# thobotics/geometry_rl

Measured on AMD Instinct MI355X. Metric: policy-update steps/sec, HEPi 4096 envs x 128 steps, higher is better.
Workload: dtype f32 storage/accumulate, bf16x3 products (three bf16 MFMAs per f32 product)

## Files before the change

### geometry_rl_amd/csrc/edge_conv16.hip

```cpp
#include "grl_tile16.h"
#include "grl_wimg.h"
#include <cstdlib>

namespace {

constexpr int C = 64, O = 16;

constexpr int E16_WAVES = 4, E16_THREADS = 64 * E16_WAVES;
constexpr int E16_WGS = 3;
constexpr int LD1 = WI_LD1, LD2 = WI_LD2;

struct Edge16Params {
  const st_t* x_in;
  const float* pos_src;
  const float* pos_dst;
  const int* rowptr;
  const int* e_src;
  const int* e_dst;
  const int* erow;
  const float* grid, *W1, *b1, *W2, *b2, *Wk;
  int n_anchor, n_edges, dim;
  int anchor_is_dst;
  int per_edge;
  int npw;
  const int* split;
  const void* wimg;
};

GRL_DEVINL void load_w16(ChainW16& s, const Edge16Params& p) {
  if (p.wimg) {
    copy_image<E16_THREADS>(&s, p.wimg, (int)sizeof(ChainW16));
    return;
  }
  stage16<14, 32, E16_THREADS>(s.W1h, s.W1l, p.W1, LD1);
  stage16<64, 64, E16_THREADS>(s.W2h, s.W2l, p.W2, LD2);
  stage16<64, 64, E16_THREADS>(s.Wkh, s.Wkl, p.Wk, LD2);
  stage_chain16_small<E16_THREADS>(s, p.b1, p.b2, p.grid);
}

template <int KS, bool FENCED = true, class Epi>
GRL_DEVINL void group16(const unsigned short* whi, const unsigned short* wlo, const bf16x8 (&xh)[KS], const bf16x8 (&xl)[KS], f32x4v acc,
                        Epi&& epi) {
  bf16x8 wh[KS], wl[KS];
#pragma unroll
  for (int s = 0; s < KS; ++s) {
    wh[s] = *reinterpret_cast<const bf16x8*>(whi + 32 * s);
    GRL_LO(wl[s] = *reinterpret_cast<const bf16x8*>(wlo + 32 * s);)
  }
  if (FENCED) __builtin_amdgcn_sched_barrier(0);
#pragma unroll
  for (int s = 0; s < KS; ++s) {
    acc = mfma16(wh[s], xh[s], acc);
    GRL_LO(acc = mfma16(wl[s], xh[s], acc);)
    GRL_LO(acc = mfma16(wh[s], xl[s], acc);)
  }
  epi(acc);
  if (FENCED) __builtin_amdgcn_sched_barrier(0);
}


template <class KEpi>
GRL_DEVINL void chain16(const ChainW16& w, float a, float b, int r, int g, KEpi&& k_epi) {
  const float aa = a * a, ab = a * b, bb = b * b;
  float4 phi;
  if (g == 0) phi = make_float4(a, b, aa, ab);
  else if (g == 1) phi = make_float4(ab, bb, aa * a, aa * b);
  else if (g == 2) phi = make_float4(ab * a, ab * b, ab * a, ab * b);
  else phi = make_float4(bb * a, bb * b, 0.f, 0.f);
  bf16x8 ph[1], pl[1];
  split_pair(phi, make_float4(0.f, 0.f, 0.f, 0.f), ph[0], pl[0]);
  float4 g1[4], g2[4];
#pragma unroll
  for (int nt = 0; nt < 4; ++nt) {
    const float4 bq = *reinterpret_cast<const float4*>(w.b1s + 16 * nt + 4 * g);
    group16<1>(w.W1h + (16 * nt + r) * LD1 + 8 * g, w.W1l + (16 * nt + r) * LD1 + 8 * g, ph, pl, f32x4v{bq.x, bq.y, bq.z, bq.w},
               [&](const f32x4v& acc) { g1[nt] = gelu4(v4(acc)); });
  }
  bf16x8 xh[2], xl[2];
  split_pair(g1[0], g1[1], xh[0], xl[0]);
  split_pair(g1[2], g1[3], xh[1], xl[1]);
  __builtin_amdgcn_sched_barrier(0);
#pragma unroll
  for (int nt = 0; nt < 4; ++nt) {
    const float4 bq = *reinterpret_cast<const float4*>(w.b2s + 16 * nt + 4 * g);
    group16<2>(w.W2h + (16 * nt + r) * LD2 + 8 * g, w.W2l + (16 * nt + r) * LD2 + 8 * g, xh, xl, f32x4v{bq.x, bq.y, bq.z, bq.w},
               [&](const f32x4v& acc) { g2[nt] = gelu4(v4(acc)); });
  }
  bf16x8 yh[2], yl[2];
  split_pair(g2[0], g2[1], yh[0], yl[0]);
  split_pair(g2[2], g2[3], yh[1], yl[1]);
  __builtin_amdgcn_sched_barrier(0);
#pragma unroll
  for (int nt = 0; nt < 4; ++nt)
    group16<2>(w.Wkh + (16 * nt + r) * LD2 + 8 * g, w.Wkl + (16 * nt + r) * LD2 + 8 * g, yh, yl, f32x4v{0.f, 0.f, 0.f, 0.f},
               [&](const f32x4v& acc) { k_epi(nt, v4(acc)); });
}

#if GRL_PREC
struct ChainRegs {
  bf16x8 w2[4][2], wk[4][2];
  GRL_LO(bf16x8 w2l[4][2]; bf16x8 wkl[4][2];)
};
GRL_DEVINL void chain_regs_load(ChainRegs& cr, const ChainW16& w, int r, int g) {
#pragma unroll
  for (int nt = 0; nt < 4; ++nt) {
#pragma unroll
    for (int s = 0; s < 2; ++s) {
      cr.w2[nt][s] = *reinterpret_cast<const bf16x8*>(w.W2h + (16 * nt + r) * LD2 + 8 * g + 32 * s);
      cr.wk[nt][s] = *reinterpret_cast<const bf16x8*>(w.Wkh + (16 * nt + r) * LD2 + 8 * g + 32 * s);
      GRL_LO(cr.w2l[nt][s] = *reinterpret_cast<const bf16x8*>(w.W2l + (16 * nt + r) * LD2 + 8 * g + 32 * s);)
      GRL_LO(cr.wkl[nt][s] = *reinterpret_cast<const bf16x8*>(w.Wkl + (16 * nt + r) * LD2 + 8 * g + 32 * s);)
    }
  }
}
template <class KEpi>
GRL_DEVINL void chain16_resident(const ChainRegs& cr, const ChainW16& w, float a, float b, int r, int g, KEpi&& k_epi) {
  __builtin_amdgcn_sched_barrier(0);
  float4 b1q[4], b2q[4];
  bf16x8 w1[4];
  GRL_LO(bf16x8 w1l[4];)
#pragma unroll
  for (int nt = 0; nt < 4; ++nt) {
    w1[nt] = *reinterpret_cast<const bf16x8*>(w.W1h + (16 * nt + r) * LD1 + 8 * g);
    GRL_LO(w1l[nt] = *reinterpret_cast<const bf16x8*>(w.W1l + (16 * nt + r) * LD1 + 8 * g);)
    b1q[nt] = *reinterpret_cast<const float4*>(w.b1s + 16 * nt + 4 * g);
    b2q[nt] = *reinterpret_cast<const float4*>(w.b2s + 16 * nt + 4 * g);
  }
  const float aa = a * a, ab = a * b, bb = b * b;
  float4 phi;
  if (g == 0) phi = make_float4(a, b, aa, ab);
  else if (g == 1) phi = make_float4(ab, bb, aa * a, aa * b);
  else if (g == 2) phi = make_float4(ab * a, ab * b, ab * a, ab * b);
  else phi = make_float4(bb * a, bb * b, 0.f, 0.f);
  bf16x8 ph, pl;
  split_pair(phi, make_float4(0.f, 0.f, 0.f, 0.f), ph, pl);
  f32x4v c[4];
  float4 g1[4], g2[4];
#pragma unroll
  for (int nt = 0; nt < 4; ++nt) c[nt] = mfma16(w1[nt], ph, f32x4v{b1q[nt].x, b1q[nt].y, b1q[nt].z, b1q[nt].w});
#if !GRL_PREC
#pragma unroll
  for (int nt = 0; nt < 4; ++nt) c[nt] = mfma16(w1l[nt], ph, c[nt]);
#pragma unroll
  for (int nt = 0; nt < 4; ++nt) c[nt] = mfma16(w1[nt], pl, c[nt]);
#endif
#pragma unroll
  for (int nt = 0; nt < 4; ++nt) g1[nt] = gelu4(v4(c[nt]));
  bf16x8 xh[2], xl[2];
  split_pair(g1[0], g1[1], xh[0], xl[0]);
  split_pair(g1[2], g1[3], xh[1], xl[1]);
#pragma unroll
  for (int nt = 0; nt < 4; ++nt) c[nt] = f32x4v{b2q[nt].x, b2q[nt].y, b2q[nt].z, b2q[nt].w};
#pragma unroll
  for (int s = 0; s < 2; ++s) {
#pragma unroll
    for (int nt = 0; nt < 4; ++nt) c[nt] = mfma16(cr.w2[nt][s], xh[s], c[nt]);
#if !GRL_PREC
#pragma unroll
    for (int nt = 0; nt < 4; ++nt) c[nt] = mfma16(cr.w2l[nt][s], xh[s], c[nt]);
#pragma unroll
    for (int nt = 0; nt < 4; ++nt) c[nt] = mfma16(cr.w2[nt][s], xl[s], c[nt]);
#endif
  }
#pragma unroll
  for (int nt = 0; nt < 4; ++nt) g2[nt] = gelu4(v4(c[nt]));
  bf16x8 yh[2], yl[2];
  split_pair(g2[0], g2[1], yh[0], yl[0]);
  split_pair(g2[2], g2[3], yh[1], yl[1]);
#pragma unroll
  for (int nt = 0; nt < 4; ++nt) c[nt] = f32x4v{0.f, 0.f, 0.f, 0.f};
#pragma unroll
  for (int s = 0; s < 2; ++s) {
#pragma unroll
    for (int nt = 0; nt < 4; ++nt) c[nt] = mfma16(cr.wk[nt][s], yh[s], c[nt]);
#if !GRL_PREC
#pragma unroll
    for (int nt = 0; nt < 4; ++nt) c[nt] = mfma16(cr.wkl[nt][s], yh[s], c[nt]);
#pragma unroll
    for (int nt = 0; nt < 4; ++nt) c[nt] = mfma16(cr.wk[nt][s], yl[s], c[nt]);
#endif
  }
#pragma unroll
  for (int nt = 0; nt < 4; ++nt) k_epi(nt, v4(c[nt]));
  __builtin_amdgcn_sched_barrier(0);
}
#define E16_CHAIN(S, A, B, R, G, EPI) chain16_resident(cregs, S, A, B, R, G, EPI)
#else
#define E16_CHAIN chain16
#endif
constexpr int NPW_MAX = 16;

template <int MODE>
__global__ __launch_bounds__(E16_THREADS, E16_WGS) void edge16_kernel(Edge16Params p, st_t* __restrict__ out, const st_t* __restrict__ dres) {
  extern __shared__ __attribute__((aligned(16))) float smem_raw[];
  ChainW16& s = *reinterpret_cast<ChainW16*>(smem_raw);
  load_w16(s, p);
  __syncthreads();
  const int lane = threadIdx.x & 63, wave = threadIdx.x >> 6, r = lane & 15, g = lane >> 4;
  const float gx = s.grid_s[3 * r], gy = s.grid_s[3 * r + 1], gz = s.grid_s[3 * r + 2];
#if GRL_PREC
  ChainRegs cregs;
  chain_regs_load(cregs, s, r, g);
#endif
  const int* e_other = p.anchor_is_dst ? p.e_src : p.e_dst;
  const float* pos_anchor = p.anchor_is_dst ? p.pos_dst : p.pos_src;
  const float* pos_other = p.anchor_is_dst ? p.pos_src : p.pos_dst;
  const int NPW = p.split ? NPW_MAX : p.npw;
  const int n_chunks = (p.n_anchor + NPW - 1) / NPW;
  const int slot = blockIdx.x * E16_WAVES + wave;
  const int n_lo = p.split ? p.split[slot] : 0, n_hi = p.split ? p.split[slot + 1] : p.n_anchor;
  for (int it = 0;; ++it) {
    int n0, nn;
    if (p.split) {
      n0 = n_lo + it * NPW_MAX;
      if (n0 >= n_hi) break;
      nn = min(NPW_MAX, n_hi - n0);
    } else {
      const int chunk = slot + it * (int)gridDim.x * E16_WAVES;
      if (chunk >= n_chunks) break;
      n0 = chunk * NPW;
      nn = min(NPW, p.n_anchor - n0);
    }
    const int rp = p.rowptr[n0 + min(lane, nn)];
    const int an = n0 + min(lane, nn - 1);
    const float pax = pos_anchor[3 * an], pay = pos_anchor[3 * an + 1], paz = pos_anchor[3 * an + 2];
    const int E0 = __builtin_amdgcn_readlane(rp, 0), E1 = __builtin_amdgcn_readlane(rp, nn);
    int node = 0;
    int node_end = __builtin_amdgcn_readlane(rp, 1);
    float4 acc[4];
#pragma unroll
    for (int t = 0; t < 4; ++t) acc[t] = make_float4(0.f, 0.f, 0.f, 0.f);
    auto flush = [&](int j) {
      if (MODE == 2) return;
      st_t* o = out + ((size_t)(n0 + j) * O + r) * C + 4 * g;
#pragma unroll
      for (int t = 0; t < 4; ++t) {
        float4 v = acc[t];
        if (MODE == 1 && dres) v = f4_add_pk(v, ld4(dres + ((size_t)(n0 + j) * O + r) * C + 4 * g + 16 * t));
        st4(o + 16 * t, v);
        acc[t] = make_float4(0.f, 0.f, 0.f, 0.f);
      }
    };
    for (int eb = E0; eb < E1; eb += 64) {
      const int ee = min(eb + lane, E1 - 1);
      const int oth = e_other[ee];
      const int xrow = p.per_edge ? (p.erow ? p.erow[ee] : ee) : oth;
      const float pox = pos_other[3 * oth], poy = pos_other[3 * oth + 1], poz = pos_other[3 * oth + 2];
      const int nb = min(64, E1 - eb);
#pragma unroll 1
      for (int k = 0; k < nb; ++k) {
        const int e = eb + k;
        while (e >= node_end) {
          flush(node);
          ++node;
          node_end = __builtin_amdgcn_readlane(rp, node + 1);
        }
        const int row_in = __builtin_amdgcn_readlane(xrow, k);
        const st_t* xs = p.x_in + ((size_t)row_in * O + r) * C + 4 * g;
        float4 xv[4];
#pragma unroll
        for (int t = 0; t < 4; ++t)
          xv[t] = ld4(xs + 16 * t);
        float dx = __builtin_bit_cast(float, __builtin_amdgcn_readlane(__builtin_bit_cast(int, pox), k)) -
                   __builtin_bit_cast(float, __builtin_amdgcn_readlane(__builtin_bit_cast(int, pax), node));
        float dy = __builtin_bit_cast(float, __builtin_amdgcn_readlane(__builtin_bit_cast(int, poy), k)) -
                   __builtin_bit_cast(float, __builtin_amdgcn_readlane(__builtin_bit_cast(int, pay), node));
        float dz = __builtin_bit_cast(float, __builtin_amdgcn_readlane(__builtin_bit_cast(int, poz), k)) -
                   __builtin_bit_cast(float, __builtin_amdgcn_readlane(__builtin_bit_cast(int, paz), node));
        if (!p.anchor_is_dst) { dx = -dx; dy = -dy; dz = -dz; }
        if (p.dim == 2) dz = 0.f;
        const float a = dx * gx + dy * gy + dz * gz;
        dx -= a * gx; dy -= a * gy; dz -= a * gz;
        const float b = sqrtf(dx * dx + dy * dy + dz * dz);
        st_t* mrow = MODE == 2 ? out + ((size_t)e * O + r) * C + 4 * g : nullptr;
        E16_CHAIN(s, a, b, r, g, [&](int nt, const float4& kq) {
          const float4 m = f4_mul_pk(kq, xv[nt]);
          if (MODE == 2) st4(mrow + 16 * nt, m);
          else acc[nt] = f4_add_pk(acc[nt], m);
        });
      }
    }
    for (; node < nn; ++node) flush(node);
  }
}

struct Stage16 {
  unsigned short Ah[STG], Al[STG];
  unsigned short Bh[STG], Bl[STG];
};
struct Bwd16Smem {
  Edge16Image img;
  Stage16 st[4];
};
constexpr int BWD16_PARTIAL = 64 * 14 + 64 + 64 * 64 + 64 + 64 * 64;

template <int NTK>
struct RFrags {
  bf16x8 ah[2], al[2], bh[NTK], bl[NTK];
};
template <int NTK>
GRL_DEVINL void rowred_load(const Stage16& st, int lane, RFrags<NTK>& f) {
#pragma unroll
  for (int t = 0; t < 2; ++t) {
    f.ah[t] = tr_frag(st.Ah, t, lane);
    GRL_LO(f.al[t] = tr_frag(st.Al, t, lane);)
  }
#pragma unroll
  for (int t = 0; t < NTK; ++t) {
    f.bh[t] = tr_frag(st.Bh, t, lane);
    GRL_LO(f.bl[t] = tr_frag(st.Bl, t, lane);)
  }
}
template <int NTK>
GRL_DEVINL void rowred_mma(const RFrags<NTK>& f, f32x16 (&acc)[2][NTK]) {
#pragma unroll
  for (int tn = 0; tn < 2; ++tn)
#pragma unroll
    for (int tk = 0; tk < NTK; ++tk) {
      mfma32_acc(f.ah[tn], f.bh[tk], acc[tn][tk]);
      GRL_LO(mfma32_acc(f.al[tn], f.bh[tk], acc[tn][tk]);)
      GRL_LO(mfma32_acc(f.ah[tn], f.bl[tk], acc[tn][tk]);)
    }
}

GRL_DEVINL void gelu_both4_pk(const float4& x, float4& gv, float4& gpv) {
  v2f g0, g1, d0, d1;
  gelu_pair<true>(v2f{x.x, x.y}, g0, d0);
  gelu_pair<true>(v2f{x.z, x.w}, g1, d1);
  gv = make_float4(g0.x, g0.y, g1.x, g1.y);
  gpv = make_float4(d0.x, d0.y, d1.x, d1.y);
}
#ifdef GRL_B16_PHASE
__device__ unsigned long long g_b16phase[16];
#define B16_PH(i) do { const unsigned long long t_ = __builtin_amdgcn_s_memtime(); ph_[i] += t_ - tl_; tl_ = t_; } while (0)
#else
#define B16_PH(i)
#endif
struct Bwd16Params {
  Edge16Params e;
  const st_t* x_src;
  const st_t* dres;
  st_t* dx_src;
  float* partial;
  const int* split;
};

__global__ __launch_bounds__(256, 1) void edge_bwd16_kernel(Bwd16Params bp) {
  extern __shared__ __attribute__((aligned(16))) float smem_raw[];
  Bwd16Smem& sm = *reinterpret_cast<Bwd16Smem*>(smem_raw);
  const Edge16Params& p = bp.e;
  if (p.wimg) {
    copy_image<256>(&sm.img, p.wimg, (int)sizeof(Edge16Image));
  } else {
    stage16<14, 32, 256>(sm.img.w.W1h, sm.img.w.W1l, p.W1, LD1);
    stage16<64, 64, 256>(sm.img.w.W2h, sm.img.w.W2l, p.W2, LD2);
    stage16<64, 64, 256>(sm.img.w.Wkh, sm.img.w.Wkl, p.Wk, LD2);
    stage16<64, 64, 256, true>(sm.img.WkTh, sm.img.WkTl, p.Wk, LD2);
    stage16<64, 64, 256, true>(sm.img.W2Th, sm.img.W2Tl, p.W2, LD2);
    stage_chain16_small<256>(sm.img.w, p.b1, p.b2, p.grid);
  }
  const int lane = threadIdx.x & 63, wave = threadIdx.x >> 6, r = lane & 15, g = lane >> 4;
  Stage16& st = sm.st[wave];
  for (int i = lane; i < STG / 2; i += 64) {
    reinterpret_cast<unsigned*>(st.Ah)[i] = 0u; reinterpret_cast<unsigned*>(st.Al)[i] = 0u;
    reinterpret_cast<unsigned*>(st.Bh)[i] = 0u; reinterpret_cast<unsigned*>(st.Bl)[i] = 0u;
  }
  __syncthreads();
  const ChainW16& w = sm.img.w;
  const float gx = w.grid_s[3 * r], gy = w.grid_s[3 * r + 1], gz = w.grid_s[3 * r + 2];
  const bool g0 = g == 0, g1_ = g == 1, g2_ = g == 2;

#if GRL_PREC
  struct LayerFrags { bf16x8 h[4][2]; };
  auto lf_load = [&](LayerFrags& f, const unsigned short* img) {
#pragma unroll
    for (int nt = 0; nt < 4; ++nt)
#pragma unroll
      for (int s_ = 0; s_ < 2; ++s_) f.h[nt][s_] = *reinterpret_cast<const bf16x8*>(img + (16 * nt + r) * LD2 + 8 * g + 32 * s_);
  };
  LayerFrags bufA, bufB;
  lf_load(bufA, w.W2h);
  lf_load(bufB, w.Wkh);
#else
  struct LayerFrags { bf16x8 h[4][2], l[4][2]; };
  auto lf_load = [&](LayerFrags& f, const unsigned short* imh, const unsigned short* iml) {
#pragma unroll
    for (int nt = 0; nt < 4; ++nt)
#pragma unroll
      for (int s_ = 0; s_ < 2; ++s_) {
        f.h[nt][s_] = *reinterpret_cast<const bf16x8*>(imh + (16 * nt + r) * LD2 + 8 * g + 32 * s_);
        f.l[nt][s_] = *reinterpret_cast<const bf16x8*>(iml + (16 * nt + r) * LD2 + 8 * g + 32 * s_);
      }
  };
  LayerFrags buf;
  lf_load(buf, w.W2h, w.W2l);
#endif
  f32x16 accK[2][2], accA[2][2], accB[2][1];
#pragma unroll
  for (int a_ = 0; a_ < 2; ++a_) {
    accB[a_][0] = zero16();
#pragma unroll
    for (int b_ = 0; b_ < 2; ++b_) { accK[a_][b_] = zero16(); accA[a_][b_] = zero16(); }
  }
  float4 db2[4];
#pragma unroll
  for (int t = 0; t < 4; ++t) db2[t] = make_float4(0.f, 0.f, 0.f, 0.f);

#ifdef GRL_B16_PHASE
  unsigned long long ph_[12] = {0}, tl_ = __builtin_amdgcn_s_memtime();
#endif
  const int NPW = bp.split ? NPW_MAX : p.npw;
  const int slot = blockIdx.x * 4 + wave;
  const int n_lo = bp.split ? bp.split[slot] : 0, n_hi = bp.split ? bp.split[slot + 1] : p.n_anchor;
  const int n_chunks = (p.n_anchor + NPW - 1) / NPW;
#pragma unroll 1
  for (int it = 0;; ++it) {
    int n0, nn;
    if (bp.split) {
      n0 = n_lo + it * NPW_MAX;
      if (n0 >= n_hi) break;
      nn = min(NPW_MAX, n_hi - n0);
    } else {
      const int chunk = slot + it * (int)gridDim.x * 4;
// ... 287 lines not shown
#if GRL_PREC
        materialise();
#endif
        bf16x8 kh[2], kl[2];
        RFrags<2> rf;
        layer64(4, yh, yl, [&](int nt, const f32x4v& c) { acc[nt] = f4_add_pk(acc[nt], f4_mul_pk(v4(c), dv[nt])); },
                [&]() {
                  split_pair(f4_mul_pk(dv[0], xv[0]), f4_mul_pk(dv[1], xv[1]), kh[0], kl[0]);
                  split_pair(f4_mul_pk(dv[2], xv[2]), f4_mul_pk(dv[3], xv[3]), kh[1], kl[1]);
                  stage_put<2>(st.Ah, st.Al, kh, kl, r, g);
                  stage_put<2>(st.Bh, st.Bl, yh, yl, r, g);
                  rowred_load<2>(st, lane, rf);
                });
        B16_PH(3);
        bf16x8 zh[2], zl[2];
        {
          float4 dz2[4];
          layer64(8, kh, kl,
                  [&](int nt, const f32x4v& c) {
                    dz2[nt] = f4_mul_pk(v4(c), gp2[nt]);
                    db2[nt] = f4_add_pk(db2[nt], dz2[nt]);
                  },
                  [&]() {
                    rowred_mma<2>(rf, accK);
                    split_pair(dz2[0], dz2[1], zh[0], zl[0]);
                    split_pair(dz2[2], dz2[3], zh[1], zl[1]);
                  });
        }
        B16_PH(4);
        stage_put<2>(st.Ah, st.Al, zh, zl, r, g);
        stage_put<2>(st.Bh, st.Bl, xh, xl, r, g);
        rowred_load<2>(st, lane, rf);
        bf16x8 uh[2], ul[2];
        {
          float4 dz1[4];
          layer64(12, zh, zl, [&](int nt, const f32x4v& c) { dz1[nt] = f4_mul_pk(v4(c), gp1[nt]); },
                  [&]() {
                    rowred_mma<2>(rf, accA);
                    split_pair(dz1[0], dz1[1], uh[0], ul[0]);
                    split_pair(dz1[2], dz1[3], uh[1], ul[1]);
                  });
        }
        B16_PH(5);
        stage_put<2>(st.Ah, st.Al, uh, ul, r, g);
        {
          const u32x4 h4 = __builtin_bit_cast(u32x4, ph[0]);
          *reinterpret_cast<uint2*>(st.Bh + stg_off(r, g)) = make_uint2(h4[0], h4[1]);
          *reinterpret_cast<uint2*>(st.Bh + stg_off(r, 4 + g)) = make_uint2(0u, 0u);
#if !GRL_PREC
          const u32x4 l4 = __builtin_bit_cast(u32x4, pl[0]);
          *reinterpret_cast<uint2*>(st.Bl + stg_off(r, g)) = make_uint2(l4[0], l4[1]);
          *reinterpret_cast<uint2*>(st.Bl + stg_off(r, 4 + g)) = make_uint2(0u, 0u);
#endif
        }
        B16_PH(6);
#undef BAR
      }
    }
    flush(node);
    skip_empty_run(node + 1, nn);
  }

  {
    RFrags<1> rf1;
    rowred_load<1>(st, lane, rf1);
    rowred_mma<1>(rf1, accB);
  }
#ifdef GRL_B16_PHASE
  if (lane == 0 && wave == 0)
    for (int i = 0; i < 12; ++i) atomicAdd(&g_b16phase[i], ph_[i]);
#endif
  constexpr int NACC = 10 * 16 + 16;
  float* fold = smem_raw;
  acc_drain(accB[0][0], accB[1][0], accA[0][0], accA[0][1], accA[1][0], accA[1][1], accK[0][0], accK[0][1], accK[1][0], accK[1][1]);
  auto visit = [&](auto&& f) {
    int k = 0;
#pragma unroll
    for (int a_ = 0; a_ < 2; ++a_) {
#pragma unroll
      for (int i = 0; i < 16; ++i) accB[a_][0][i] = f(accB[a_][0][i], k++);
#pragma unroll
      for (int b_ = 0; b_ < 2; ++b_)
#pragma unroll
        for (int i = 0; i < 16; ++i) { accA[a_][b_][i] = f(accA[a_][b_][i], k++); accK[a_][b_][i] = f(accK[a_][b_][i], k++); }
    }
#pragma unroll
    for (int t = 0; t < 4; ++t) {
      db2[t].x = f(db2[t].x, k++); db2[t].y = f(db2[t].y, k++); db2[t].z = f(db2[t].z, k++); db2[t].w = f(db2[t].w, k++);
    }
  };
  __syncthreads();
  if (wave & 1) visit([&](float v_, int k) { fold[((wave >> 1) * NACC + k) * 64 + lane] = v_; return v_; });
  __syncthreads();
  if (!(wave & 1)) visit([&](float v_, int k) { return v_ + fold[((wave >> 1) * NACC + k) * 64 + lane]; });
  __syncthreads();
  if (wave == 2) visit([&](float v_, int k) { fold[k * 64 + lane] = v_; return v_; });
  __syncthreads();
  if (wave != 0) return;
  visit([&](float v_, int k) { return v_ + fold[k * 64 + lane]; });
  const int j = lane & 31, hh = lane >> 5;
  float* out = bp.partial + (size_t)blockIdx.x * BWD16_PARTIAL;
  float* oW1 = out, *ob1 = out + 64 * 14, *oW2 = ob1 + 64, *ob2 = oW2 + 64 * 64, *oWk = ob2 + 64;
#pragma unroll
  for (int nt = 0; nt < 2; ++nt)
#pragma unroll
    for (int rho = 0; rho < 16; ++rho) {
      const int n = 32 * nt + (rho & 3) + 8 * (rho >> 2) + 4 * hh;
      if (j < 14) oW1[n * 14 + j] = accB[nt][0][rho];
      if (j == 14) ob1[n] = accB[nt][0][rho];
#pragma unroll
      for (int kt = 0; kt < 2; ++kt) {
        oW2[n * 64 + 32 * kt + j] = accA[nt][kt][rho];
        oWk[n * 64 + 32 * kt + j] = accK[nt][kt][rho];
      }
    }
#pragma unroll
  for (int t = 0; t < 4; ++t) {
    float v[4] = {db2[t].x, db2[t].y, db2[t].z, db2[t].w};
#pragma unroll
    for (int u = 0; u < 4; ++u) {
      float x = v[u];
      x += __shfl_xor(x, 1, 64); x += __shfl_xor(x, 2, 64); x += __shfl_xor(x, 4, 64); x += __shfl_xor(x, 8, 64);
      if (r == 0) ob2[16 * t + 4 * g + u] = x;
    }
  }
}

}

extern "C" {

#if !GRL_PREC
static_assert(E16_WAVES == 4, "grl_edge_fwd_slots (edge_conv.hip) counts four wave slots per workgroup");
int grl_edge_fwd_chunk_nodes(int n_dst) {
  if (n_dst < 0) return 256 * E16_WGS;
  const int npw = n_dst / (4 * 256 * E16_WAVES * E16_WGS);
  return npw < 1 ? 1 : (npw > NPW_MAX ? NPW_MAX : npw);
}
int grl_edge_bwd_chunk_nodes(int n_src) {
  const int npw = n_src / (4 * 1024);
  return npw < 1 ? 1 : (npw > NPW_MAX ? NPW_MAX : npw);
}
#else
int grl_edge_fwd_chunk_nodes(int n_dst);
int grl_edge_bwd_chunk_nodes(int n_src);
#endif

int GRL_ENTRY(grl_edge16_launch)(int mode, const st_t* x_in, const float* pos_src, const float* pos_dst, const int* rowptr, const int* e_src,
                                 const int* e_dst, const int* erow, int per_edge, int n_anchor, int n_edges, int anchor_is_dst,
                                 const float* grid, int dim, const float* W1, const float* b1, const float* W2, const float* b2,
                                 const float* Wk, st_t* out, const st_t* dres, const int* split, int n_slots, const void* wimg,
                                 hipStream_t stream) {
  if (n_anchor <= 0) return 0;
  int npw = grl_edge_fwd_chunk_nodes(n_anchor);
  Edge16Params p{x_in, pos_src, pos_dst, rowptr, e_src, e_dst, erow, grid, W1, b1, W2, b2, Wk, n_anchor, n_edges, dim, anchor_is_dst,
                 per_edge, npw, (mode == 0 && split && n_slots >= E16_WAVES && n_slots % E16_WAVES == 0) ? split : nullptr, wimg};
  const int n_chunks = (n_anchor + npw - 1) / npw;
  int blocks = p.split ? n_slots / E16_WAVES : (n_chunks + E16_WAVES - 1) / E16_WAVES;
  int cap = 256 * E16_WGS;
  if (blocks > cap && !p.split) blocks = cap;
  if (blocks < 1) blocks = 1;
  const size_t smem = sizeof(ChainW16);
  GRL_ONCE(hipFuncSetAttribute((const void*)edge16_kernel<0>, hipFuncAttributeMaxDynamicSharedMemorySize, (int)sizeof(ChainW16));
           hipFuncSetAttribute((const void*)edge16_kernel<2>, hipFuncAttributeMaxDynamicSharedMemorySize, (int)sizeof(ChainW16)));
  if (mode == 0) hipLaunchKernelGGL(edge16_kernel<0>, dim3(blocks), dim3(E16_THREADS), smem, stream, p, out, dres);
  else if (mode == 1) return -4;
  else hipLaunchKernelGGL(edge16_kernel<2>, dim3(blocks), dim3(E16_THREADS), smem, stream, p, out, dres);
  GRL_CHECK_LAUNCH();
  return 0;
}

int GRL_ENTRY(grl_edge_bwd16_launch)(const st_t* x_src, const st_t* dmsg, const float* pos_src, const float* pos_dst, const int* rowptr_s,
                                     const int* src_s, const int* dst_s, const int* erow, int per_edge, int n_src, int n_edges,
                                     const float* grid, int dim, const float* W1, const float* b1, const float* W2, const float* b2,
                                     const float* Wk, const st_t* dres, st_t* dx_src, float* partial, int blocks, const int* split,
                                     const void* wimg, hipStream_t stream) {
  const int npw = grl_edge_bwd_chunk_nodes(n_src);
  Bwd16Params bp{{dmsg, pos_src, pos_dst, rowptr_s, src_s, dst_s, erow, grid, W1, b1, W2, b2, Wk, n_src, n_edges, dim, 0, per_edge, npw,
                  nullptr, wimg},
                 x_src, dres, dx_src, partial, split};
  static_assert(sizeof(Bwd16Smem) > 80 * 1024, "edge_bwd16_kernel must not share a CU with a second workgroup");
  GRL_ONCE(hipFuncSetAttribute((const void*)edge_bwd16_kernel, hipFuncAttributeMaxDynamicSharedMemorySize, (int)sizeof(Bwd16Smem)));
  hipLaunchKernelGGL(edge_bwd16_kernel, dim3(blocks), dim3(256), sizeof(Bwd16Smem), stream, bp);
  GRL_CHECK_LAUNCH();
  return 0;
}

#if defined(GRL_B16_PHASE)
int GRL_ENTRY(grl_edge_bwd16_phase_read)(unsigned long long* out16, int reset) {
  hipMemcpyFromSymbol(out16, HIP_SYMBOL(g_b16phase), sizeof(unsigned long long) * 16);
  if (reset) { unsigned long long z[16] = {0}; hipMemcpyToSymbol(HIP_SYMBOL(g_b16phase), z, sizeof(z)); }
  return 0;
}
#endif

}
```

### geometry_rl_amd/csrc/grl_common.h

```cpp
#pragma once
#include <hip/hip_runtime.h>
#include <stdint.h>

typedef float f32x16 __attribute__((ext_vector_type(16)));

#define GRL_DEVINL __device__ __forceinline__

#define GRL_LD(K) ((K) + 4)

GRL_DEVINL f32x16 mfma32(float a, float b, f32x16 c) { return __builtin_amdgcn_mfma_f32_32x32x2f32(a, b, c, 0, 0, 0); }

GRL_DEVINL f32x16 zero16() {
  f32x16 z;
#pragma unroll
  for (int i = 0; i < 16; ++i) z[i] = 0.f;
  return z;
}

template <int K>
GRL_DEVINL void mma_wx(const float* wrow, const float4 (&x)[K / 8], f32x16& acc) {
#pragma unroll
  for (int t = 0; t < K / 8; ++t) {
    const float4 w = *reinterpret_cast<const float4*>(wrow + 8 * t);
    acc = mfma32(w.x, x[t].x, acc);
    acc = mfma32(w.y, x[t].y, acc);
    acc = mfma32(w.z, x[t].z, acc);
    acc = mfma32(w.w, x[t].w, acc);
  }
}

template <int N>
GRL_DEVINL void mma_wTy(const float* wcol, int ldw, const float4 (&y)[N / 8], f32x16& acc) {
#pragma unroll
  for (int t = 0; t < N / 8; ++t) {
    const float* p = wcol + (8 * t) * ldw;
    acc = mfma32(p[0], y[t].x, acc);
    acc = mfma32(p[ldw], y[t].y, acc);
    acc = mfma32(p[2 * ldw], y[t].z, acc);
    acc = mfma32(p[3 * ldw], y[t].w, acc);
  }
}

template <int R>
GRL_DEVINL void mma_tn(const float* pcol, int ldp, const float* qcol, int ldq, f32x16& acc) {
#pragma unroll
  for (int t = 0; t < R / 8; ++t) {
    const float* p = pcol + (8 * t) * ldp;
    const float* q = qcol + (8 * t) * ldq;
    acc = mfma32(p[0], q[0], acc);
    acc = mfma32(p[ldp], q[ldq], acc);
    acc = mfma32(p[2 * ldp], q[2 * ldq], acc);
    acc = mfma32(p[3 * ldp], q[3 * ldq], acc);
  }
}

GRL_DEVINL void acc_to_frag(const f32x16& a, float4& f0, float4& f1, float4& f2, float4& f3) {
  f0 = make_float4(a[0], a[1], a[2], a[3]);
  f1 = make_float4(a[4], a[5], a[6], a[7]);
  f2 = make_float4(a[8], a[9], a[10], a[11]);
  f3 = make_float4(a[12], a[13], a[14], a[15]);
}

#ifndef GRL_PREC
#define GRL_PREC 0
#endif
GRL_DEVINL float gelu_logistic(float x) {
  const float w = x * fmaf(x * x, -0.07056f * 1.44269504088896f, -1.5976f * 1.44269504088896f);
  return x * __builtin_amdgcn_rcpf(1.f + __builtin_amdgcn_exp2f(w));
}
GRL_DEVINL void gelu_logistic_both(float x, float& g, float& gp) {
  const float x2 = x * x;
  const float w = x * fmaf(x2, -0.07056f * 1.44269504088896f, -1.5976f * 1.44269504088896f);
  const float s = __builtin_amdgcn_rcpf(1.f + __builtin_amdgcn_exp2f(w));
  g = x * s;
  gp = fmaf(fmaf(-s, s, s), x * fmaf(x2, 3.f * 0.07056f, 1.5976f), s);
}
typedef float v2f __attribute__((ext_vector_type(2)));
GRL_DEVINL v2f fma2(v2f a, v2f b, v2f c) { return __builtin_elementwise_fma(a, b, c); }
GRL_DEVINL v2f splat2(float a) { return v2f{a, a}; }
GRL_DEVINL void gelu_logistic_pair(v2f x, v2f& g) {
  const v2f w = x * fma2(x * x, splat2(-0.07056f * 1.44269504088896f), splat2(-1.5976f * 1.44269504088896f));
  v2f a;
  a.x = __builtin_amdgcn_exp2f(w.x);
  a.y = __builtin_amdgcn_exp2f(w.y);
  a = a + splat2(1.f);
  v2f s_;
  s_.x = __builtin_amdgcn_rcpf(a.x);
  s_.y = __builtin_amdgcn_rcpf(a.y);
  g = x * s_;
}
GRL_DEVINL void gelu_logistic_both_pair(v2f x, v2f& g, v2f& gp) {
  const v2f x2 = x * x;
  const v2f w = x * fma2(x2, splat2(-0.07056f * 1.44269504088896f), splat2(-1.5976f * 1.44269504088896f));
  v2f a;
  a.x = __builtin_amdgcn_exp2f(w.x);
  a.y = __builtin_amdgcn_exp2f(w.y);
  a = a + splat2(1.f);
  v2f s_;
  s_.x = __builtin_amdgcn_rcpf(a.x);
  s_.y = __builtin_amdgcn_rcpf(a.y);
  g = x * s_;
  gp = fma2(fma2(-s_, s_, s_), x * fma2(x2, splat2(3.f * 0.07056f), splat2(1.5976f)), s_);
}
template <bool WITH_GRAD> GRL_DEVINL void gelu_pair_as(v2f x, v2f& g, v2f& gp);
template <bool WITH_GRAD>
GRL_DEVINL void gelu_pair(v2f x, v2f& g, v2f& gp) {
#if GRL_PREC
  if (WITH_GRAD) gelu_logistic_both_pair(x, g, gp);
  else gelu_logistic_pair(x, g);
  return;
#endif
  gelu_pair_as<WITH_GRAD>(x, g, gp);
}
template <bool WITH_GRAD>
GRL_DEVINL void gelu_pair_as(v2f x, v2f& g, v2f& gp) {
  const float kp = 0.3275911f * 0.70710678118654752440f;
  v2f t, e;
  t.x = __builtin_amdgcn_rcpf(fmaf(fabsf(x.x), kp, 1.0f));
  t.y = __builtin_amdgcn_rcpf(fmaf(fabsf(x.y), kp, 1.0f));
  if (WITH_GRAD) {
    const v2f arg = fma2(x * x, splat2(-0.72134752044448170368f), splat2(-1.32574806473615910f));
    e.x = __builtin_amdgcn_exp2f(arg.x);
    e.y = __builtin_amdgcn_exp2f(arg.y);
    v2f poly = fma2(t, splat2(1.33027442959f), splat2(-1.82125597911f));
    poly = fma2(poly, t, splat2(1.78147793657f));
    poly = fma2(poly, t, splat2(-0.35656378125f));
    poly = fma2(poly, t, splat2(0.31938153026f));
    const v2f hq = (poly * t) * e;
    const v2f w = splat2(0.5f) - hq;
    v2f ws;
    ws.x = copysignf(w.x, x.x);
    ws.y = copysignf(w.y, x.y);
    const v2f cdf = ws + splat2(0.5f);
    g = x * cdf;
    gp = fma2(x, e, cdf);
  } else {
    const v2f arg = (x * x) * splat2(-0.72134752044448170368f);
    e.x = __builtin_amdgcn_exp2f(arg.x);
    e.y = __builtin_amdgcn_exp2f(arg.y);
    v2f poly = fma2(t, splat2(0.5307027145f), splat2(-0.7265760135f));
    poly = fma2(poly, t, splat2(0.7107068705f));
    poly = fma2(poly, t, splat2(-0.142248368f));
    poly = fma2(poly, t, splat2(0.127414796f));
    const v2f hq = (poly * t) * e;
    g.x = fmaf(-fabsf(x.x), hq.x, fmaxf(x.x, 0.f));
    g.y = fmaf(-fabsf(x.y), hq.y, fmaxf(x.y, 0.f));
  }
}
GRL_DEVINL float gelu_val(float x) {
#if GRL_PREC
  return gelu_logistic(x);
#endif
  const float t = __builtin_amdgcn_rcpf(fmaf(fabsf(x), 0.3275911f * 0.70710678118654752440f, 1.0f));
  const float e = __builtin_amdgcn_exp2f((x * x) * -0.72134752044448170368f);
  float poly = fmaf(t, 0.5307027145f, -0.7265760135f);
  poly = fmaf(poly, t, 0.7107068705f);
  poly = fmaf(poly, t, -0.142248368f);
  poly = fmaf(poly, t, 0.127414796f);
  return fmaf(-fabsf(x), (poly * t) * e, fmaxf(x, 0.f));
}
#ifndef GRL_GELU4_SCALAR
#define GRL_GELU4_SCALAR 0
#endif
GRL_DEVINL float4 gelu4(float4 x) {
#if GRL_GELU4_SCALAR
  return make_float4(gelu_val(x.x), gelu_val(x.y), gelu_val(x.z), gelu_val(x.w));
#endif
  v2f g0, g1, d0, d1;
  gelu_pair<false>(v2f{x.x, x.y}, g0, d0);
  gelu_pair<false>(v2f{x.z, x.w}, g1, d1);
  return make_float4(g0.x, g0.y, g1.x, g1.y);
}
GRL_DEVINL void gelu_both_as(float x, float& g, float& gp);
GRL_DEVINL void gelu_both(float x, float& g, float& gp) {
#if GRL_PREC
  gelu_logistic_both(x, g, gp);
  return;
#endif
  gelu_both_as(x, g, gp);
}
GRL_DEVINL void gelu_both_as(float x, float& g, float& gp) {
  const float t = __builtin_amdgcn_rcpf(fmaf(fabsf(x), 0.3275911f * 0.70710678118654752440f, 1.0f));
  const float e = __builtin_amdgcn_exp2f(fmaf(x * x, -0.72134752044448170368f, -1.32574806473615910f));
  float poly = fmaf(t, 1.33027442959f, -1.82125597911f);
  poly = fmaf(poly, t, 1.78147793657f);
  poly = fmaf(poly, t, -0.35656378125f);
  poly = fmaf(poly, t, 0.31938153026f);
  const float hq = (poly * t) * e;
  const float cdf = copysignf(0.5f - hq, x) + 0.5f;
  g = x * cdf;
  gp = fmaf(x, e, cdf);
}
GRL_DEVINL void gelu_both4(float4 x, float4& g, float4& gp) {
  gelu_both(x.x, g.x, gp.x);
  gelu_both(x.y, g.y, gp.y);
  gelu_both(x.z, g.z, gp.z);
  gelu_both(x.w, g.w, gp.w);
}
GRL_DEVINL float4 gelu_grad4(float4 x) {
  float4 g, gp;
  gelu_both4(x, g, gp);
  return gp;
}
GRL_DEVINL float gelu_f(float x) {
  v2f g, gp;
  gelu_pair<false>(v2f{x, x}, g, gp);
  return g.x;
}
GRL_DEVINL float gelu_grad_f(float x) {
  float g, gp;
  gelu_both(x, g, gp);
  return gp;
}
GRL_DEVINL float gelu_exact_f(float x) {
  v2f g, gp;
  gelu_pair_as<false>(v2f{x, x}, g, gp);
  return g.x;
}
GRL_DEVINL float gelu_exact_grad_f(float x) {
  float g, gp;
  gelu_both_as(x, g, gp);
  return gp;
}

typedef float f32x4n __attribute__((ext_vector_type(4)));
GRL_DEVINL float4 load_nt4(const float* p) {
  const f32x4n v = __builtin_nontemporal_load(reinterpret_cast<const f32x4n*>(p));
  return make_float4(v.x, v.y, v.z, v.w);
}
GRL_DEVINL void store_nt4(float* p, const float4& v) {
  __builtin_nontemporal_store(f32x4n{v.x, v.y, v.z, v.w}, reinterpret_cast<f32x4n*>(p));
}
GRL_DEVINL float4 f4_mul(float4 a, float4 b) { return make_float4(a.x * b.x, a.y * b.y, a.z * b.z, a.w * b.w); }
GRL_DEVINL float4 f4_add(float4 a, float4 b) { return make_float4(a.x + b.x, a.y + b.y, a.z + b.z, a.w + b.w); }
GRL_DEVINL float4 f4_mul_pk(float4 a, float4 b) {
  const v2f lo = v2f{a.x, a.y} * v2f{b.x, b.y}, hi = v2f{a.z, a.w} * v2f{b.z, b.w};
  return make_float4(lo.x, lo.y, hi.x, hi.y);
}
GRL_DEVINL float4 f4_add_pk(float4 a, float4 b) {
  const v2f lo = v2f{a.x, a.y} + v2f{b.x, b.y}, hi = v2f{a.z, a.w} + v2f{b.z, b.w};
  return make_float4(lo.x, lo.y, hi.x, hi.y);
}
GRL_DEVINL float4 f4_scale(float4 a, float s) { return make_float4(a.x * s, a.y * s, a.z * s, a.w * s); }

GRL_DEVINL void stage_matrix(float* dst, const float* __restrict__ src, int rows, int K, int ld) {
  for (int idx = threadIdx.x; idx < rows * K; idx += blockDim.x) {
    const int r = idx / K, c = idx - r * K;
    dst[r * ld + c] = src[idx];
  }
}

void grl_prof_begin(const char* name, hipStream_t stream);
void grl_prof_end(hipStream_t stream);
void grl_prof_begin_replay(const char* name, hipStream_t stream);
void grl_prof_end_replay(hipStream_t stream);

#include <mutex>
#define GRL_ONCE(...)                               \
  do {                                              \
    static std::once_flag grl_once_flag_;           \
    std::call_once(grl_once_flag_, [&] { __VA_ARGS__; }); \
  } while (0)

#define GRL_CHECK_LAUNCH()                       \
  do {                                           \
    hipError_t e_ = hipGetLastError();           \
    if (e_ != hipSuccess) return -1000 - (int)e_; \
  } while (0)

#if GRL_PREC
#define GRL_LO(...)
#define GRL_ENTRY(name) name##_bf16
#else
#define GRL_LO(...) __VA_ARGS__
#define GRL_ENTRY(name) name
#endif
typedef __bf16 bf16x8 __attribute__((ext_vector_type(8)));
typedef unsigned int u32x4 __attribute__((ext_vector_type(4)));

GRL_DEVINL f32x16 mfma_bf(bf16x8 a, bf16x8 b, f32x16 c) {
  return __builtin_amdgcn_mfma_f32_32x32x16_bf16(a, b, c, 0, 0, 0);
}

GRL_DEVINL unsigned pack_hi(float a, float b) {
  return __builtin_amdgcn_perm(__float_as_uint(b), __float_as_uint(a), 0x07060302u);
}
GRL_DEVINL float trunc_bf16(float a) { return __uint_as_float(__float_as_uint(a) & 0xFFFF0000u); }
GRL_DEVINL unsigned pack_rn(float a, float b) {
  typedef __bf16 bf16x2 __attribute__((ext_vector_type(2)));
  bf16x2 v = {(__bf16)a, (__bf16)b};
  return __builtin_bit_cast(unsigned, v);
}

GRL_DEVINL void split_pair(const float4& f0, const float4& f1, bf16x8& hi, bf16x8& lo) {
  u32x4 h, l;
#if GRL_PREC
  h[0] = pack_rn(f0.x, f0.y); h[1] = pack_rn(f0.z, f0.w); h[2] = pack_rn(f1.x, f1.y); h[3] = pack_rn(f1.z, f1.w);
  l[0] = l[1] = l[2] = l[3] = 0u;
#else
  h[0] = pack_hi(f0.x, f0.y); h[1] = pack_hi(f0.z, f0.w); h[2] = pack_hi(f1.x, f1.y); h[3] = pack_hi(f1.z, f1.w);
  l[0] = pack_rn(f0.x - trunc_bf16(f0.x), f0.y - trunc_bf16(f0.y));
  l[1] = pack_rn(f0.z - trunc_bf16(f0.z), f0.w - trunc_bf16(f0.w));
  l[2] = pack_rn(f1.x - trunc_bf16(f1.x), f1.y - trunc_bf16(f1.y));
  l[3] = pack_rn(f1.z - trunc_bf16(f1.z), f1.w - trunc_bf16(f1.w));
#endif
  hi = __builtin_bit_cast(bf16x8, h);
  lo = __builtin_bit_cast(bf16x8, l);
}
template <int K>
GRL_DEVINL void split_frags(const float4 (&x)[K / 8], bf16x8 (&hi)[K / 16], bf16x8 (&lo)[K / 16]) {
#pragma unroll
  for (int s = 0; s < K / 16; ++s) split_pair(x[2 * s], x[2 * s + 1], hi[s], lo[s]);
}

#if GRL_PREC
typedef unsigned short st_t;
GRL_DEVINL float ld1(const st_t* p) { return __uint_as_float((unsigned)(*p) << 16); }
GRL_DEVINL void st1(st_t* p, float v) { *p = (unsigned short)(pack_rn(v, 0.f) & 0xFFFFu); }
GRL_DEVINL float4 ld4(const st_t* p) {
  const uint2 u = *reinterpret_cast<const uint2*>(p);
  return make_float4(__uint_as_float(u.x << 16), __uint_as_float(u.x & 0xFFFF0000u), __uint_as_float(u.y << 16),
                     __uint_as_float(u.y & 0xFFFF0000u));
}
GRL_DEVINL void st4(st_t* p, const float4& v) {
  uint2 u;
  u.x = pack_rn(v.x, v.y);
  u.y = pack_rn(v.z, v.w);
  *reinterpret_cast<uint2*>(p) = u;
}
GRL_DEVINL float4 ld4_nt(const st_t* p) { return ld4(p); }
GRL_DEVINL void st4_nt(st_t* p, const float4& v) { st4(p, v); }
typedef uint2 raw4_t;
GRL_DEVINL raw4_t ld4_raw(const st_t* p) { return *reinterpret_cast<const uint2*>(p); }
GRL_DEVINL float4 widen4(const raw4_t& u) {
  return make_float4(__uint_as_float(u.x << 16), __uint_as_float(u.x & 0xFFFF0000u), __uint_as_float(u.y << 16),
                     __uint_as_float(u.y & 0xFFFF0000u));
}
#else
typedef float st_t;
GRL_DEVINL float ld1(const st_t* p) { return *p; }
GRL_DEVINL void st1(st_t* p, float v) { *p = v; }
GRL_DEVINL float4 ld4(const st_t* p) { return *reinterpret_cast<const float4*>(p); }
GRL_DEVINL void st4(st_t* p, const float4& v) { *reinterpret_cast<float4*>(p) = v; }
GRL_DEVINL float4 ld4_nt(const st_t* p) { return load_nt4(p); }
GRL_DEVINL void st4_nt(st_t* p, const float4& v) { store_nt4(p, v); }
typedef float4 raw4_t;
GRL_DEVINL raw4_t ld4_raw(const st_t* p) { return load_nt4(p); }
GRL_DEVINL float4 widen4(const raw4_t& u) { return u; }
#endif

#define GRL_LDB(K) ((K) + 8)

GRL_DEVINL void put_split_quad(unsigned short* hi, unsigned short* lo, const float4& w) {
  uint2 h, l;
#if GRL_PREC
  h.x = pack_rn(w.x, w.y); h.y = pack_rn(w.z, w.w);
  *reinterpret_cast<uint2*>(hi) = h;
  (void)lo; (void)l;
#else
  h.x = pack_hi(w.x, w.y); h.y = pack_hi(w.z, w.w);
  l.x = pack_rn(w.x - trunc_bf16(w.x), w.y - trunc_bf16(w.y));
  l.y = pack_rn(w.z - trunc_bf16(w.z), w.w - trunc_bf16(w.w));
  *reinterpret_cast<uint2*>(hi) = h;
  *reinterpret_cast<uint2*>(lo) = l;
#endif
}
template <int ROWS, int K, int KSRC, int NT>
GRL_DEVINL void stage_split(unsigned short* hi, unsigned short* lo, const float* __restrict__ src, int ld) {
  constexpr int Q = K / 4, N = ROWS * Q, IT = (N + NT - 1) / NT, G = IT < 8 ? IT : 8;
  const bool vec = KSRC % 4 == 0 && (reinterpret_cast<size_t>(src) & 15) == 0;
#pragma unroll 1
  for (int base = 0; base < IT; base += G) {
    float4 w[G];
#pragma unroll
    for (int g = 0; g < G; ++g) {
      const int idx = threadIdx.x + (base + g) * NT;
      const int r = idx / Q, pq = idx - r * Q, q = pq & 3;
      const int k = ((4 * pq) & ~15) + ((q == 1) ? 8 : (q == 2) ? 4 : 4 * q);
      w[g] = make_float4(0.f, 0.f, 0.f, 0.f);
      if (idx < N) {
        const float* sp = src + (size_t)r * KSRC + k;
        if (vec) {
          w[g] = *reinterpret_cast<const float4*>(sp);
        } else {
          w[g].x = k < KSRC ? sp[0] : 0.f; w[g].y = k + 1 < KSRC ? sp[1] : 0.f;
          w[g].z = k + 2 < KSRC ? sp[2] : 0.f; w[g].w = k + 3 < KSRC ? sp[3] : 0.f;
        }
      }
    }
#pragma unroll
    for (int g = 0; g < G; ++g) {
      const int idx = threadIdx.x + (base + g) * NT;
      const int r = idx / Q, pq = idx - r * Q;
      if (idx < N) put_split_quad(hi + r * ld + 4 * pq, lo + r * ld + 4 * pq, w[g]);
    }
  }
}
template <int NT>
GRL_DEVINL void stage_split_T(unsigned short* hi, unsigned short* lo, const float* __restrict__ src, int ld) {
  constexpr int N = 64 * 16, IT = (N + NT - 1) / NT;
  float4 w[IT];
#pragma unroll
  for (int g = 0; g < IT; ++g) {
    const int idx = threadIdx.x + g * NT, k = idx & 63, pq = idx >> 6, q = pq & 3;
    const int n = ((4 * pq) & ~15) + ((q == 1) ? 8 : (q == 2) ? 4 : 4 * q);
    w[g] = make_float4(0.f, 0.f, 0.f, 0.f);
    if (idx < N) w[g] = make_float4(src[n * 64 + k], src[(n + 1) * 64 + k], src[(n + 2) * 64 + k], src[(n + 3) * 64 + k]);
  }
#pragma unroll
  for (int g = 0; g < IT; ++g) {
    const int idx = threadIdx.x + g * NT, k = idx & 63, pq = idx >> 6;
    if (idx < N) put_split_quad(hi + k * ld + 4 * pq, lo + k * ld + 4 * pq, w[g]);
  }
}

template <int K>
struct WFrags { bf16x8 h[K / 16], l[K / 16]; };
template <int K>
GRL_DEVINL void load_wfrags(WFrags<K>& w, const unsigned short* whi, const unsigned short* wlo) {
#pragma unroll
  for (int s = 0; s < K / 16; ++s) {
    w.h[s] = *reinterpret_cast<const bf16x8*>(whi + 16 * s);
    GRL_LO(w.l[s] = *reinterpret_cast<const bf16x8*>(wlo + 16 * s);)
  }
}
template <int K, class Epi>
GRL_DEVINL void mma_wx_bf_fenced(const unsigned short* whi, const unsigned short* wlo, const bf16x8 (&xh)[K / 16],
                                 const bf16x8 (&xl)[K / 16], f32x16 acc, Epi&& epilogue) {
  WFrags<K> w;
  load_wfrags<K>(w, whi, wlo);
  __builtin_amdgcn_sched_barrier(0);
#pragma unroll
  for (int s = 0; s < K / 16; ++s) {
    acc = mfma_bf(w.h[s], xh[s], acc);
    GRL_LO(acc = mfma_bf(w.l[s], xh[s], acc);)
    GRL_LO(acc = mfma_bf(w.h[s], xl[s], acc);)
  }
  epilogue(acc);
  __builtin_amdgcn_sched_barrier(0);
}

GRL_DEVINL void adam_element(float g, float& p, float& m, float& v, float b1, float b2, float eps, float lr_bc1, float bc2_sqrt) {
#pragma clang fp contract(off)
  const float mi = fmaf(1.f - b1, g, b1 * m);
  const float vi = fmaf(g, (1.f - b2) * g, b2 * v);
  m = mi;
  v = vi;
  const float denom = sqrtf(vi) / bc2_sqrt + eps;
  p = fmaf(-lr_bc1, mi / denom, p);
}
```

Baseline: 330.0.

## Use packed bf16 splits, specialize anchor direction and flat dim, asm relu in gelu

Replaces the scalar hi/lo bf16 split in the edge chain with a packed v2f subtraction variant. It also hardcodes anchor_is_dst=true for non-MODE-1 kernels, skips loading z coordinates when dim==2, and uses an inline-asm v_max for the relu term in gelu. The host launcher now rejects anchor_is_dst==0 with an error code, which drops support for that path. The asm relu takes an unused extra operand, apparently to enforce scheduling order. This trims per-edge ALU and load work at the cost of lost generality.

```diff
diff --git a/geometry_rl_amd/csrc/edge_conv16.hip b/geometry_rl_amd/csrc/edge_conv16.hip
--- a/geometry_rl_amd/csrc/edge_conv16.hip
+++ b/geometry_rl_amd/csrc/edge_conv16.hip
@@ -68,7 +68,7 @@
   else if (g == 2) phi = make_float4(ab * a, ab * b, ab * a, ab * b);
   else phi = make_float4(bb * a, bb * b, 0.f, 0.f);
   bf16x8 ph[1], pl[1];
-  split_pair(phi, make_float4(0.f, 0.f, 0.f, 0.f), ph[0], pl[0]);
+  split_pair_pk(phi, make_float4(0.f, 0.f, 0.f, 0.f), ph[0], pl[0]);
   float4 g1[4], g2[4];
 #pragma unroll
   for (int nt = 0; nt < 4; ++nt) {
@@ -77,8 +77,8 @@
                [&](const f32x4v& acc) { g1[nt] = gelu4(v4(acc)); });
   }
   bf16x8 xh[2], xl[2];
-  split_pair(g1[0], g1[1], xh[0], xl[0]);
-  split_pair(g1[2], g1[3], xh[1], xl[1]);
+  split_pair_pk(g1[0], g1[1], xh[0], xl[0]);
+  split_pair_pk(g1[2], g1[3], xh[1], xl[1]);
   __builtin_amdgcn_sched_barrier(0);
 #pragma unroll
   for (int nt = 0; nt < 4; ++nt) {
@@ -87,8 +87,8 @@
                [&](const f32x4v& acc) { g2[nt] = gelu4(v4(acc)); });
   }
   bf16x8 yh[2], yl[2];
-  split_pair(g2[0], g2[1], yh[0], yl[0]);
-  split_pair(g2[2], g2[3], yh[1], yl[1]);
+  split_pair_pk(g2[0], g2[1], yh[0], yl[0]);
+  split_pair_pk(g2[2], g2[3], yh[1], yl[1]);
   __builtin_amdgcn_sched_barrier(0);
 #pragma unroll
   for (int nt = 0; nt < 4; ++nt)
@@ -202,9 +202,11 @@
   ChainRegs cregs;
   chain_regs_load(cregs, s, r, g);
 #endif
-  const int* e_other = p.anchor_is_dst ? p.e_src : p.e_dst;
-  const float* pos_anchor = p.anchor_is_dst ? p.pos_dst : p.pos_src;
-  const float* pos_other = p.anchor_is_dst ? p.pos_src : p.pos_dst;
+  const bool anchor_is_dst = MODE == 1 ? p.anchor_is_dst != 0 : true;
+  const int* e_other = anchor_is_dst ? p.e_src : p.e_dst;
+  const float* pos_anchor = anchor_is_dst ? p.pos_dst : p.pos_src;
+  const float* pos_other = anchor_is_dst ? p.pos_src : p.pos_dst;
+  const bool flat = p.dim == 2;
   const int NPW = p.split ? NPW_MAX : p.npw;
   const int n_chunks = (p.n_anchor + NPW - 1) / NPW;
   const int slot = blockIdx.x * E16_WAVES + wave;
@@ -223,7 +225,7 @@
     }
     const int rp = p.rowptr[n0 + min(lane, nn)];
     const int an = n0 + min(lane, nn - 1);
-    const float pax = pos_anchor[3 * an], pay = pos_anchor[3 * an + 1], paz = pos_anchor[3 * an + 2];
+    const float pax = pos_anchor[3 * an], pay = pos_anchor[3 * an + 1], paz = flat ? 0.f : pos_anchor[3 * an + 2];
     const int E0 = __builtin_amdgcn_readlane(rp, 0), E1 = __builtin_amdgcn_readlane(rp, nn);
     int node = 0;
     int node_end = __builtin_amdgcn_readlane(rp, 1);
@@ -245,7 +247,7 @@
       const int ee = min(eb + lane, E1 - 1);
       const int oth = e_other[ee];
       const int xrow = p.per_edge ? (p.erow ? p.erow[ee] : ee) : oth;
-      const float pox = pos_other[3 * oth], poy = pos_other[3 * oth + 1], poz = pos_other[3 * oth + 2];
+      const float pox = pos_other[3 * oth], poy = pos_other[3 * oth + 1], poz = flat ? 0.f : pos_other[3 * oth + 2];
       const int nb = min(64, E1 - eb);
 #pragma unroll 1
       for (int k = 0; k < nb; ++k) {
@@ -267,8 +269,7 @@
                    __builtin_bit_cast(float, __builtin_amdgcn_readlane(__builtin_bit_cast(int, pay), node));
         float dz = __builtin_bit_cast(float, __builtin_amdgcn_readlane(__builtin_bit_cast(int, poz), k)) -
                    __builtin_bit_cast(float, __builtin_amdgcn_readlane(__builtin_bit_cast(int, paz), node));
-        if (!p.anchor_is_dst) { dx = -dx; dy = -dy; dz = -dz; }
-        if (p.dim == 2) dz = 0.f;
+        if (!anchor_is_dst) { dx = -dx; dy = -dy; dz = -dz; }
         const float a = dx * gx + dy * gy + dz * gz;
         dx -= a * gx; dy -= a * gy; dz -= a * gz;
         const float b = sqrtf(dx * dx + dy * dy + dz * dz);
@@ -862,6 +863,7 @@
                                  const float* Wk, st_t* out, const st_t* dres, const int* split, int n_slots, const void* wimg,
                                  hipStream_t stream) {
   if (n_anchor <= 0) return 0;
+  if (!anchor_is_dst) return -4;
   int npw = grl_edge_fwd_chunk_nodes(n_anchor);
   Edge16Params p{x_in, pos_src, pos_dst, rowptr, e_src, e_dst, erow, grid, W1, b1, W2, b2, Wk, n_anchor, n_edges, dim, anchor_is_dst,
                  per_edge, npw, (mode == 0 && split && n_slots >= E16_WAVES && n_slots % E16_WAVES == 0) ? split : nullptr, wimg};
diff --git a/geometry_rl_amd/csrc/grl_common.h b/geometry_rl_amd/csrc/grl_common.h
--- a/geometry_rl_amd/csrc/grl_common.h
+++ b/geometry_rl_amd/csrc/grl_common.h
@@ -101,6 +101,11 @@
   s_.y = __builtin_amdgcn_rcpf(a.y);
   g = x * s_;
   gp = fma2(fma2(-s_, s_, s_), x * fma2(x2, splat2(3.f * 0.07056f), splat2(1.5976f)), s_);
+}
+GRL_DEVINL float relu_f(float x, float after) {
+  float d;
+  asm("v_max_f32 %0, 0, %1" : "=v"(d) : "v"(x), "v"(after));
+  return d;
 }
 template <bool WITH_GRAD> GRL_DEVINL void gelu_pair_as(v2f x, v2f& g, v2f& gp);
 template <bool WITH_GRAD>
@@ -143,8 +148,8 @@
     poly = fma2(poly, t, splat2(-0.142248368f));
     poly = fma2(poly, t, splat2(0.127414796f));
     const v2f hq = (poly * t) * e;
-    g.x = fmaf(-fabsf(x.x), hq.x, fmaxf(x.x, 0.f));
-    g.y = fmaf(-fabsf(x.y), hq.y, fmaxf(x.y, 0.f));
+    g.x = fmaf(-fabsf(x.x), hq.x, relu_f(x.x, t.x));
+    g.y = fmaf(-fabsf(x.y), hq.y, relu_f(x.y, t.y));
   }
 }
 GRL_DEVINL float gelu_val(float x) {
@@ -157,7 +162,7 @@
   poly = fmaf(poly, t, 0.7107068705f);
   poly = fmaf(poly, t, -0.142248368f);
   poly = fmaf(poly, t, 0.127414796f);
-  return fmaf(-fabsf(x), (poly * t) * e, fmaxf(x, 0.f));
+  return fmaf(-fabsf(x), (poly * t) * e, relu_f(x, t));
 }
 #ifndef GRL_GELU4_SCALAR
 #define GRL_GELU4_SCALAR 0
@@ -306,6 +311,19 @@
 #endif
   hi = __builtin_bit_cast(bf16x8, h);
   lo = __builtin_bit_cast(bf16x8, l);
+}
+GRL_DEVINL void split_pair_pk(const float4& f0, const float4& f1, bf16x8& hi, bf16x8& lo) {
+#if GRL_PREC
+  split_pair(f0, f1, hi, lo);
+#else
+  u32x4 h, l;
+  h[0] = pack_hi(f0.x, f0.y); h[1] = pack_hi(f0.z, f0.w); h[2] = pack_hi(f1.x, f1.y); h[3] = pack_hi(f1.z, f1.w);
+  const v2f d0 = v2f{f0.x, f0.y} - v2f{trunc_bf16(f0.x), trunc_bf16(f0.y)}, d1 = v2f{f0.z, f0.w} - v2f{trunc_bf16(f0.z), trunc_bf16(f0.w)};
+  const v2f d2 = v2f{f1.x, f1.y} - v2f{trunc_bf16(f1.x), trunc_bf16(f1.y)}, d3 = v2f{f1.z, f1.w} - v2f{trunc_bf16(f1.z), trunc_bf16(f1.w)};
+  l[0] = pack_rn(d0.x, d0.y); l[1] = pack_rn(d1.x, d1.y); l[2] = pack_rn(d2.x, d2.y); l[3] = pack_rn(d3.x, d3.y);
+  hi = __builtin_bit_cast(bf16x8, h);
+  lo = __builtin_bit_cast(bf16x8, l);
+#endif
 }
 template <int K>
 GRL_DEVINL void split_frags(const float4 (&x)[K / 8], bf16x8 (&hi)[K / 16], bf16x8 (&lo)[K / 16]) {
```

New measurement: 332.3, median of 6. No clear change (+0.7%).
